# MayDomine/Burst-Attention

Hardware: NVIDIA H100
Metric: attention fwd+bwd TFLOPS/s (bs=1, H=32, d=128, bf16; seq in config, default 262144 on N > 1 GPUs, 65536 on one), aggregate over GPUs (higher is better)
Workload: dtype bf16

## Files before the change

burst-attention_b200/csrc/fwd_sm90.cu:

```cuda
#include <math.h>
#include <stdlib.h>

#include "host_common.h"
#include "sm90_ptx.cuh"

namespace ba {

constexpr int kBlockM = 128;
constexpr int kBlockN = 128;
constexpr int kKStages = 2;
constexpr int kVStages = 2;
constexpr int kBoxBytes = 128 * 64 * 2;
constexpr int kFwdThreads = 384;

struct FwdParams {
  float* o_acc;
  int64_t oacc_sb, oacc_ss, oacc_sh;
  float* lse;
  int64_t lse_sb, lse_sh;
  void* o_out;
  int64_t oout_sb, oout_ss, oout_sh;
  int B, Sq, Sk, H;
  int G;
  float scale_log2;
  const float* bias;
  int64_t bias_sb, bias_sh;
  int causal;
  int causal_off;
  int load_state;
  int store_lowp;
};

struct __align__(8) FwdBarriers {
  uint64_t q_full;
  uint64_t k_full[kKStages], k_empty[kKStages];
  uint64_t b_full[kKStages];
  uint64_t v_full[kVStages], v_empty[kVStages];
};

template <int kD>
struct FwdLayout {
  static_assert(kD == 64 || kD == 128, "head dim 64 or 128");
  static constexpr uint32_t kTileB = 128 * kD * 2;
  static constexpr int kBoxes = kD / 64;
  static constexpr uint32_t kOffQ = 0;
  static constexpr uint32_t kOffK = kTileB;
  static constexpr uint32_t kOffV = kOffK + kKStages * kTileB;
  static constexpr uint32_t kOffBias = kOffV + kVStages * kTileB;
  static constexpr uint32_t kOffBars = kOffBias + kKStages * kBlockN * 4;
  static constexpr int kSmemBytes = kOffBars + 256 ;
  static_assert(kSmemBytes <= 232448, "forward kernel exceeds 227 KiB of shared memory");
};

__device__ __forceinline__ int fwd_trip_count(int r0, const FwdParams& p) {
  if (r0 >= p.Sq) return 0;
  int r_last = min(r0 + 63, p.Sq - 1);
  int max_limit = p.causal ? min(r_last + p.causal_off, p.Sk - 1) : p.Sk - 1;
  return max_limit < 0 ? 0 : max_limit / kBlockN + 1;
}

template <bool kBF16, int kD, bool kBias>
__global__ void __launch_bounds__(kFwdThreads, 1)
fwd_chunk_kernel(const __grid_constant__ CUtensorMap tmQ, const __grid_constant__ CUtensorMap tmK,
                 const __grid_constant__ CUtensorMap tmV, const FwdParams p) {
  extern __shared__ __align__(1024) uint8_t smem_raw[];
  uint8_t* smem = smem_raw;
  if ((smem_u32(smem) & 1023u) != 0) __trap();
  using L = FwdLayout<kD>;
  constexpr uint32_t kTileBytes = L::kTileB;
  constexpr int kBoxes = L::kBoxes, kOReg = kD / 2;
  uint8_t* sQ = smem + L::kOffQ;
  uint8_t* sK = smem + L::kOffK;
  uint8_t* sV = smem + L::kOffV;
  float* sBias = reinterpret_cast<float*>(smem + L::kOffBias);
  FwdBarriers* bars = reinterpret_cast<FwdBarriers*>(smem + L::kOffBars);

  const int warp = __shfl_sync(0xffffffffu, threadIdx.x >> 5, 0);
  const int lane = threadIdx.x & 31;
  const int h = blockIdx.y, b = blockIdx.z;
  const int row0 = (p.causal ? (int)(gridDim.x - 1 - blockIdx.x) : (int)blockIdx.x) * kBlockM;
  const int n_tiles = max(fwd_trip_count(row0, p), fwd_trip_count(row0 + 64, p));

  if (threadIdx.x == 0) {
    tma_prefetch_desc(&tmQ);
    tma_prefetch_desc(&tmK);
    tma_prefetch_desc(&tmV);
    mbar_init(&bars->q_full, 1);
    for (int i = 0; i < kKStages; ++i) {
      mbar_init(&bars->k_full[i], 1);
      mbar_init(&bars->k_empty[i], 8);
      mbar_init(&bars->b_full[i], 1);
    }
    for (int i = 0; i < kVStages; ++i) {
      mbar_init(&bars->v_full[i], 1);
      mbar_init(&bars->v_empty[i], 8);
    }
    fence_mbar_init();
  }
  __syncthreads();

  if (warp < 4) {
    reg_alloc_dec<40>();
    if (warp != 0) return;
    const int hk = h / p.G;
    if (lane == 0) {
      mbar_arrive_expect_tx(&bars->q_full, kTileBytes);
      for (int half = 0; half < kBoxes; ++half)
        tma_load_4d(sQ + half * kBoxBytes, &tmQ, &bars->q_full, half * 64, h, row0, b);
    }
    for (int i = 0; i < n_tiles; ++i) {
      const int ks = i % kKStages, kph = (i / kKStages) & 1;
      mbar_wait(&bars->k_empty[ks], kph ^ 1);
      if (lane == 0) {
        mbar_arrive_expect_tx(&bars->k_full[ks], kTileBytes);
        for (int half = 0; half < kBoxes; ++half)
          tma_load_4d(sK + ks * kTileBytes + half * kBoxBytes, &tmK, &bars->k_full[ks], half * 64, hk,
                      i * kBlockN, b);
      }
      if constexpr (kBias) {
#pragma unroll
        for (int j = 0; j < 4; ++j) {
          const int key = i * kBlockN + lane + 32 * j;
          float x = 0.f;
          if (key < p.Sk) x = __ldg(p.bias + (int64_t)b * p.bias_sb + (int64_t)h * p.bias_sh + key) * kLog2e;
          sBias[ks * kBlockN + lane + 32 * j] = x;
        }
        __syncwarp();
        if (lane == 0) mbar_arrive(&bars->b_full[ks]);
      }
      if (lane == 0) {
        const int vs = i % kVStages, vph = (i / kVStages) & 1;
        mbar_wait(&bars->v_empty[vs], vph ^ 1);
        mbar_arrive_expect_tx(&bars->v_full[vs], kTileBytes);
        for (int half = 0; half < kBoxes; ++half)
          tma_load_4d(sV + vs * kTileBytes + half * kBoxBytes, &tmV, &bars->v_full[vs], half * 64, hk,
                      i * kBlockN, b);
      }
      __syncwarp();
    }
    return;
  }

  reg_alloc_inc<232>();
  const int wg = (threadIdx.x >> 7) - 1;
  const int w = warp & 3, g = lane >> 2, t = lane & 3;
  const int r_lo = row0 + wg * 64 + 16 * w + g;
  const int rows[2] = {r_lo, r_lo + 8};
  const int n_mine = fwd_trip_count(row0 + wg * 64, p);
  const float scale_log2 = p.scale_log2;
  int limit[2];
#pragma unroll
  for (int r = 0; r < 2; ++r) limit[r] = p.causal ? min(rows[r] + p.causal_off, p.Sk - 1) : p.Sk - 1;
  const int limit_min = min(limit[0], limit[1]);

  float o[kOReg];
  float m[2] = {-INFINITY, -INFINITY}, l[2] = {0.f, 0.f};
#pragma unroll
  for (int i = 0; i < kOReg; ++i) o[i] = 0.f;
  if (p.load_state) {
#pragma unroll
    for (int r = 0; r < 2; ++r) {
      if (rows[r] >= p.Sq) continue;
      const float lse_prev = p.lse[(int64_t)b * p.lse_sb + (int64_t)h * p.lse_sh + rows[r]];
      if (lse_prev != -INFINITY) {
        m[r] = lse_prev * kLog2e;
        l[r] = t == 0 ? 1.f : 0.f;
      }
      const float* src = p.o_acc + (int64_t)b * p.oacc_sb + (int64_t)rows[r] * p.oacc_ss + (int64_t)h * p.oacc_sh;
#pragma unroll
      for (int c = 0; c < kD / 8; ++c) {
        const float2 f = __ldg(reinterpret_cast<const float2*>(src + 8 * c + 2 * t));
        o[4 * c + 2 * r] = f.x;
        o[4 * c + 2 * r + 1] = f.y;
      }
    }
  }

  const uint32_t q_base = smem_u32(sQ) + wg * 64 * 128;
  mbar_wait(&bars->q_full, 0);
  for (int i = 0; i < n_tiles; ++i) {
    const int ks = i % kKStages, kph = (i / kKStages) & 1;
    const int vs = i % kVStages, vph = (i / kVStages) & 1;
    const bool work = i < n_mine;
    mbar_wait(&bars->k_full[ks], kph);
    float sc[64];
    if (work) {
      const uint32_t k_base = smem_u32(sK + ks * kTileBytes);
      wgmma_fence();
#pragma unroll
      for (int kk = 0; kk < kD / 16; ++kk) {
        const uint32_t off = (kk >> 2) * kBoxBytes + (kk & 3) * 32;
        wgmma_ss_n128<kBF16, 0, 0>(sc, make_desc(q_base + off, 16, 1024), make_desc(k_base + off, 16, 1024),
                                   kk > 0 ? 1u : 0u);
      }
      wgmma_commit();
      wgmma_wait<0>();
      fence_regs<64>(sc);
      const int key0 = i * kBlockN;
      if constexpr (kBias) {
        mbar_wait(&bars->b_full[ks], kph);
        const float* bias = sBias + ks * kBlockN;
#pragma unroll
        for (int c = 0; c < 16; ++c) {
          const float2 bb = *reinterpret_cast<const float2*>(bias + 8 * c + 2 * t);
#pragma unroll
          for (int r = 0; r < 2; ++r) {
            sc[4 * c + 2 * r] = fmaf(sc[4 * c + 2 * r], scale_log2, bb.x);
            sc[4 * c + 2 * r + 1] = fmaf(sc[4 * c + 2 * r + 1], scale_log2, bb.y);
          }
        }
      } else {
#pragma unroll
        for (int j = 0; j < 64; ++j) sc[j] *= scale_log2;
      }
      if (key0 + kBlockN - 1 > limit_min) {
#pragma unroll
        for (int c = 0; c < 16; ++c)
#pragma unroll
          for (int e = 0; e < 4; ++e)
            if (key0 + 8 * c + 2 * t + (e & 1) > limit[e >> 1]) sc[4 * c + e] = -INFINITY;
      }
    }
    __syncwarp();
    if (lane == 0) mbar_arrive(&bars->k_empty[ks]);
    if (work) {
      uint32_t pa[32];
#pragma unroll
      for (int r = 0; r < 2; ++r) {
        float mx = -INFINITY;
#pragma unroll
        for (int c = 0; c < 16; ++c) mx = fmaxf(mx, fmaxf(sc[4 * c + 2 * r], sc[4 * c + 2 * r + 1]));
        mx = fmaxf(mx, __shfl_xor_sync(0xffffffffu, mx, 1));
        mx = fmaxf(mx, __shfl_xor_sync(0xffffffffu, mx, 2));
        const float m_new = fmaxf(m[r], mx);
        const float f = (m[r] == -INFINITY) ? 0.f : ex2(m[r] - m_new);
        const float neg_m = (m_new == -INFINITY) ? 0.f : -m_new;
        m[r] = m_new;
        float sum = 0.f;
#pragma unroll
        for (int c = 0; c < 16; ++c) {
          const float p0 = ex2(sc[4 * c + 2 * r] + neg_m), p1 = ex2(sc[4 * c + 2 * r + 1] + neg_m);
          sc[4 * c + 2 * r] = p0;
          sc[4 * c + 2 * r + 1] = p1;
          sum += p0 + p1;
        }
        l[r] = l[r] * f + sum;
#pragma unroll
        for (int c = 0; c < kD / 8; ++c) {
          o[4 * c + 2 * r] *= f;
          o[4 * c + 2 * r + 1] *= f;
        }
      }
#pragma unroll
      for (int j = 0; j < 32; ++j) pa[j] = pack2<kBF16>(sc[2 * j], sc[2 * j + 1]);
      mbar_wait(&bars->v_full[vs], vph);
      const uint32_t v_base = smem_u32(sV + vs * kTileBytes);
      fence_regs<32>(pa);
      fence_regs<kOReg>(o);
      wgmma_fence();
#pragma unroll
      for (int kk = 0; kk < kBlockN / 16; ++kk) {
        const uint64_t dv = make_desc(v_base + kk * 16 * 128, kBoxBytes, 1024);
        if constexpr (kD == 128) wgmma_rs_n128<kBF16, 1>(o, pa + 4 * kk, dv, 1u);
        else wgmma_rs_n64<kBF16, 1>(o, pa + 4 * kk, dv, 1u);
      }
      wgmma_commit();
      wgmma_wait<0>();
      fence_regs<kOReg>(o);
    } else {
      mbar_wait(&bars->v_full[vs], vph);
    }
    __syncwarp();
    if (lane == 0) mbar_arrive(&bars->v_empty[vs]);
  }

#pragma unroll
  for (int r = 0; r < 2; ++r) {
    float lr = l[r];
    lr += __shfl_xor_sync(0xffffffffu, lr, 1);
    lr += __shfl_xor_sync(0xffffffffu, lr, 2);
    const int row = rows[r];
    if (row >= p.Sq) continue;
    const float inv_l = lr > 0.f ? 1.f / lr : 0.f;
    if (t == 0) p.lse[(int64_t)b * p.lse_sb + (int64_t)h * p.lse_sh + row] = lr > 0.f ? (m[r] + lg2(lr)) * kLn2 : -INFINITY;
    if (p.store_lowp) {
      uint16_t* dst = reinterpret_cast<uint16_t*>(p.o_out) + (int64_t)b * p.oout_sb + (int64_t)row * p.oout_ss +
                      (int64_t)h * p.oout_sh + 2 * t;
#pragma unroll
      for (int c = 0; c < kD / 8; ++c)
        *reinterpret_cast<uint32_t*>(dst + 8 * c) = pack2<kBF16>(o[4 * c + 2 * r] * inv_l, o[4 * c + 2 * r + 1] * inv_l);
    } else {
      float* dst = p.o_acc + (int64_t)b * p.oacc_sb + (int64_t)row * p.oacc_ss + (int64_t)h * p.oacc_sh + 2 * t;
#pragma unroll
      for (int c = 0; c < kD / 8; ++c)
        *reinterpret_cast<float2*>(dst + 8 * c) = make_float2(o[4 * c + 2 * r] * inv_l, o[4 * c + 2 * r + 1] * inv_l);
    }
  }
}


static int launch_fwd(int dtype, int D, bool bias, const CUtensorMap& tmQ, const CUtensorMap& tmK,
                      const CUtensorMap& tmV, const FwdParams& p, cudaStream_t stream) {
  const bool bf16 = dtype == BA_DTYPE_BF16;
  void (*kern)(CUtensorMap, CUtensorMap, CUtensorMap, FwdParams);
  if (bias)
    kern = D == 64 ? (bf16 ? fwd_chunk_kernel<true, 64, true> : fwd_chunk_kernel<false, 64, true>)
                   : (bf16 ? fwd_chunk_kernel<true, 128, true> : fwd_chunk_kernel<false, 128, true>);
  else
    kern = D == 64 ? (bf16 ? fwd_chunk_kernel<true, 64, false> : fwd_chunk_kernel<false, 64, false>)
                   : (bf16 ? fwd_chunk_kernel<true, 128, false> : fwd_chunk_kernel<false, 128, false>);
  const int smem = D == 64 ? FwdLayout<64>::kSmemBytes : FwdLayout<128>::kSmemBytes;
  BA_CHECK_CUDA(cudaFuncSetAttribute(kern, cudaFuncAttributeMaxDynamicSharedMemorySize, smem));
  dim3 grid((p.Sq + kBlockM - 1) / kBlockM, p.H, p.B);
  kern<<<grid, kFwdThreads, smem, stream>>>(tmQ, tmK, tmV, p);
  BA_CHECK_CUDA(cudaGetLastError());
  return BA_OK;
}

}

extern "C" int ba_fwd_chunk(ba_tensor4 q, ba_tensor4 k, ba_tensor4 v, ba_tensor4 o_acc, ba_rowstat lse,
                            ba_tensor4 o_out, int B, int Sq, int Sk, int H, int D, float scale, int mask_mode,
                            int causal_offset, int flags, int dtype, void* stream) {
  ba_rowstat none = {nullptr, 0, 0};
  return ba_fwd_chunk_bias(q, k, v, none, o_acc, lse, o_out, B, Sq, Sk, H, D, scale, mask_mode, causal_offset, flags,
                           dtype, stream);
}

extern "C" int ba_fwd_chunk_bias(ba_tensor4 q, ba_tensor4 k, ba_tensor4 v, ba_rowstat key_bias, ba_tensor4 o_acc,
                                 ba_rowstat lse, ba_tensor4 o_out, int B, int Sq, int Sk, int H, int D, float scale,
                                 int mask_mode, int causal_offset, int flags, int dtype, void* stream) {
  return ba_fwd_chunk_gqa(q, k, v, key_bias, o_acc, lse, o_out, B, Sq, Sk, H, H, D, scale, mask_mode, causal_offset,
                          flags, dtype, stream);
}

extern "C" int ba_fwd_chunk_gqa(ba_tensor4 q, ba_tensor4 k, ba_tensor4 v, ba_rowstat key_bias, ba_tensor4 o_acc,
                                ba_rowstat lse, ba_tensor4 o_out, int B, int Sq, int Sk, int H, int H_kv, int D,
                                float scale, int mask_mode, int causal_offset, int flags, int dtype, void* stream) {
  using namespace ba;
  int rc;
  if ((rc = check_chunk_args("ba_fwd_chunk", B, Sq, Sk, H, H_kv, D, scale, mask_mode, dtype))) return rc;
  BA_REQUIRE(q.ptr && k.ptr && v.ptr && lse.ptr, "ba_fwd_chunk: null q/k/v/lse");
  const bool first = flags & BA_FWD_FIRST, last = flags & BA_FWD_LAST;
  BA_REQUIRE(!last || o_out.ptr, "ba_fwd_chunk: BA_FWD_LAST needs o_out");
  BA_REQUIRE((first && last) || o_acc.ptr, "ba_fwd_chunk: fp32 state o_acc required unless FIRST|LAST");
  if (o_acc.ptr)
    BA_REQUIRE(aligned16(o_acc, 4), "ba_fwd_chunk: o_acc must be 16-byte aligned with strides multiple of 4 elements");
  if (o_out.ptr)
    BA_REQUIRE(aligned16(o_out, 2), "ba_fwd_chunk: o_out must be 16-byte aligned with strides multiple of 8 elements");

  CUtensorMap tmQ, tmK, tmV;
  const CUtensorMapDataType dt = lowp_dtype(dtype);
  if ((rc = make_tensor_map(&tmQ, q, B, Sq, H, D, dt, 2, 64, kBlockM, true))) return rc;
  if ((rc = make_tensor_map(&tmK, k, B, Sk, H_kv, D, dt, 2, 64, kBlockN, true))) return rc;
  if ((rc = make_tensor_map(&tmV, v, B, Sk, H_kv, D, dt, 2, 64, kBlockN, true))) return rc;

  FwdParams p;
  p.o_acc = static_cast<float*>(o_acc.ptr);
  p.oacc_sb = o_acc.stride_b, p.oacc_ss = o_acc.stride_s, p.oacc_sh = o_acc.stride_h;
  p.lse = lse.ptr;
  p.lse_sb = lse.stride_b, p.lse_sh = lse.stride_h;
  p.o_out = o_out.ptr;
  p.oout_sb = o_out.stride_b, p.oout_ss = o_out.stride_s, p.oout_sh = o_out.stride_h;
  p.B = B, p.Sq = Sq, p.Sk = Sk, p.H = H;
  p.G = H / H_kv;
  p.scale_log2 = scale * kLog2e;
  p.causal = mask_mode == BA_MASK_CAUSAL;
  p.causal_off = causal_offset;
  p.load_state = first ? 0 : 1;
  p.store_lowp = last ? 1 : 0;
  p.bias = key_bias.ptr, p.bias_sb = key_bias.stride_b, p.bias_sh = key_bias.stride_h;
  return launch_fwd(dtype, D, key_bias.ptr != nullptr, tmQ, tmK, tmV, p, static_cast<cudaStream_t>(stream));
}
```

burst-attention_b200/csrc/sm90_ptx.cuh:

```cuda
#pragma once
#include <cuda.h>
#include <cuda_bf16.h>
#include <cuda_fp16.h>
#include <cuda_runtime.h>
#include <stdint.h>

namespace ba {

#define BA_DEVICE __device__ __forceinline__

BA_DEVICE uint32_t smem_u32(const void* p) {
  return static_cast<uint32_t>(__cvta_generic_to_shared(p));
}
constexpr float kLog2e = 1.4426950408889634f;
constexpr float kLn2 = 0.6931471805599453f;
BA_DEVICE float ex2(float x) {
  float y;
  asm("ex2.approx.ftz.f32 %0, %1;" : "=f"(y) : "f"(x));
  return y;
}
BA_DEVICE float lg2(float x) {
  float y;
  asm("lg2.approx.ftz.f32 %0, %1;" : "=f"(y) : "f"(x));
  return y;
}
template <int N>
BA_DEVICE void reg_alloc_inc() {
  asm volatile("setmaxnreg.inc.sync.aligned.u32 %0;" ::"n"(N));
}
template <int N>
BA_DEVICE void reg_alloc_dec() {
  asm volatile("setmaxnreg.dec.sync.aligned.u32 %0;" ::"n"(N));
}

BA_DEVICE void mbar_init(uint64_t* bar, uint32_t count) {
  asm volatile("mbarrier.init.shared::cta.b64 [%0], %1;" ::"r"(smem_u32(bar)), "r"(count));
}
BA_DEVICE void fence_mbar_init() { asm volatile("fence.mbarrier_init.release.cluster;" ::: "memory"); }
BA_DEVICE void mbar_arrive(uint64_t* bar) {
  asm volatile("mbarrier.arrive.shared::cta.b64 _, [%0];" ::"r"(smem_u32(bar)) : "memory");
}
BA_DEVICE void mbar_arrive_expect_tx(uint64_t* bar, uint32_t bytes) {
  asm volatile("mbarrier.arrive.expect_tx.shared::cta.b64 _, [%0], %1;" ::"r"(smem_u32(bar)), "r"(bytes)
               : "memory");
}
BA_DEVICE bool mbar_try_wait(uint64_t* bar, uint32_t parity) {
  uint32_t ok;
  asm volatile(
      "{\n\t.reg .pred p;\n\t"
      "mbarrier.try_wait.parity.shared::cta.b64 p, [%1], %2;\n\t"
      "selp.u32 %0, 1, 0, p;\n\t}\n"
      : "=r"(ok)
      : "r"(smem_u32(bar)), "r"(parity)
      : "memory");
  return ok != 0;
}
BA_DEVICE uint64_t global_ns() {
  uint64_t t;
  asm volatile("mov.u64 %0, %%globaltimer;" : "=l"(t));
  return t;
}
BA_DEVICE void mbar_wait(uint64_t* bar, uint32_t parity) {
  if (mbar_try_wait(bar, parity)) return;
#ifdef BA_NO_WATCHDOG
  while (!mbar_try_wait(bar, parity)) {
  }
#else
  const uint64_t t0 = global_ns();
#pragma unroll 1
  for (;;) {
#pragma unroll 1
    for (int i = 0; i < 1024; ++i)
      if (mbar_try_wait(bar, parity)) return;
    if (global_ns() - t0 > 30000000000ull) break;
  }
  __trap();
#endif
}

BA_DEVICE void fence_proxy_async_smem() { asm volatile("fence.proxy.async.shared::cta;" ::: "memory"); }
BA_DEVICE void named_bar_sync(uint32_t id, uint32_t nthreads) {
  asm volatile("bar.sync %0, %1;" ::"r"(id), "r"(nthreads) : "memory");
}

BA_DEVICE void tma_prefetch_desc(const CUtensorMap* m) {
  asm volatile("prefetch.tensormap [%0];" ::"l"(reinterpret_cast<uint64_t>(m)) : "memory");
}
BA_DEVICE void tma_load_4d(void* smem_dst, const CUtensorMap* m, uint64_t* bar, int c0, int c1, int c2,
                           int c3) {
  asm volatile(
      "cp.async.bulk.tensor.4d.shared::cluster.global.mbarrier::complete_tx::bytes"
      " [%0], [%1, {%3, %4, %5, %6}], [%2];"
      :
      : "r"(smem_u32(smem_dst)), "l"(reinterpret_cast<uint64_t>(m)), "r"(smem_u32(bar)), "r"(c0), "r"(c1),
        "r"(c2), "r"(c3)
      : "memory");
}
BA_DEVICE void tma_reduce_add_4d(const CUtensorMap* m, const void* smem_src, int c0, int c1, int c2, int c3) {
  asm volatile(
      "cp.reduce.async.bulk.tensor.4d.global.shared::cta.add.tile.bulk_group [%0, {%2, %3, %4, %5}], [%1];"
      :
      : "l"(reinterpret_cast<uint64_t>(m)), "r"(smem_u32(smem_src)), "r"(c0), "r"(c1), "r"(c2), "r"(c3)
      : "memory");
}
BA_DEVICE void tma_store_commit() { asm volatile("cp.async.bulk.commit_group;" ::: "memory"); }
template <int N>
BA_DEVICE void tma_store_wait_read() {
  asm volatile("cp.async.bulk.wait_group.read %0;" ::"n"(N) : "memory");
}
template <int N>
BA_DEVICE void tma_store_wait() {
  asm volatile("cp.async.bulk.wait_group %0;" ::"n"(N) : "memory");
}

BA_DEVICE uint64_t make_desc(uint32_t smem_addr, uint32_t lbo_bytes, uint32_t sbo_bytes) {
  uint64_t d = 0;
  d |= static_cast<uint64_t>((smem_addr & 0x3FFFF) >> 4);
  d |= static_cast<uint64_t>((lbo_bytes >> 4) & 0x3FFF) << 16;
  d |= static_cast<uint64_t>((sbo_bytes >> 4) & 0x3FFF) << 32;
  d |= static_cast<uint64_t>(1) << 62;
  return d;
}

BA_DEVICE void wgmma_fence() { asm volatile("wgmma.fence.sync.aligned;" ::: "memory"); }
BA_DEVICE void wgmma_commit() { asm volatile("wgmma.commit_group.sync.aligned;" ::: "memory"); }
template <int N>
BA_DEVICE void wgmma_wait() {
  asm volatile("wgmma.wait_group.sync.aligned %0;" ::"n"(N) : "memory");
}
template <int N>
BA_DEVICE void fence_regs(float* r) {
#pragma unroll
  for (int i = 0; i < N; ++i) asm volatile("" : "+f"(r[i])::"memory");
}
template <int N>
BA_DEVICE void fence_regs(uint32_t* r) {
#pragma unroll
  for (int i = 0; i < N; ++i) asm volatile("" : "+r"(r[i])::"memory");
}

#define BA_WGMMA_ACC_64(d) "+f"(d[0]), "+f"(d[1]), "+f"(d[2]), "+f"(d[3]), "+f"(d[4]), "+f"(d[5]), "+f"(d[6]), "+f"(d[7]), "+f"(d[8]), "+f"(d[9]), "+f"(d[10]), "+f"(d[11]), "+f"(d[12]), "+f"(d[13]), "+f"(d[14]), "+f"(d[15]), "+f"(d[16]), "+f"(d[17]), "+f"(d[18]), "+f"(d[19]), "+f"(d[20]), "+f"(d[21]), "+f"(d[22]), "+f"(d[23]), "+f"(d[24]), "+f"(d[25]), "+f"(d[26]), "+f"(d[27]), "+f"(d[28]), "+f"(d[29]), "+f"(d[30]), "+f"(d[31])
#define BA_WGMMA_ACC_128(d) BA_WGMMA_ACC_64(d), "+f"(d[32]), "+f"(d[33]), "+f"(d[34]), "+f"(d[35]), "+f"(d[36]), "+f"(d[37]), "+f"(d[38]), "+f"(d[39]), "+f"(d[40]), "+f"(d[41]), "+f"(d[42]), "+f"(d[43]), "+f"(d[44]), "+f"(d[45]), "+f"(d[46]), "+f"(d[47]), "+f"(d[48]), "+f"(d[49]), "+f"(d[50]), "+f"(d[51]), "+f"(d[52]), "+f"(d[53]), "+f"(d[54]), "+f"(d[55]), "+f"(d[56]), "+f"(d[57]), "+f"(d[58]), "+f"(d[59]), "+f"(d[60]), "+f"(d[61]), "+f"(d[62]), "+f"(d[63])
#define BA_WGMMA_REGS_64 "%0,%1,%2,%3,%4,%5,%6,%7,%8,%9,%10,%11,%12,%13,%14,%15,%16,%17,%18,%19,%20,%21,%22,%23,%24,%25,%26,%27,%28,%29,%30,%31"
#define BA_WGMMA_REGS_128 BA_WGMMA_REGS_64 ",%32,%33,%34,%35,%36,%37,%38,%39,%40,%41,%42,%43,%44,%45,%46,%47,%48,%49,%50,%51,%52,%53,%54,%55,%56,%57,%58,%59,%60,%61,%62,%63"
#define BA_WGMMA_SS(N, TY, A, B, SC, TA, TB)                                                     \
  asm volatile("{\n\t.reg .pred p;\n\t"                                                        \
               "setp.ne.b32 p, %" #SC ", 0;\n\t"                                               \
               "wgmma.mma_async.sync.aligned.m64n" #N "k16.f32." TY "." TY " "                 \
               "{" BA_WGMMA_REGS_##N "}, "                                                      \
               "%" #A ", %" #B ", p, 1, 1, %" #TA ", %" #TB ";\n\t}\n"                         \
               : BA_WGMMA_ACC_##N(d)                                                            \
               : "l"(a_desc), "l"(b_desc), "r"(scale_d), "n"(kTA), "n"(kTB))
#define BA_WGMMA_RS(N, TY, A0, A1, A2, A3, B, SC, TB)                                            \
  asm volatile("{\n\t.reg .pred p;\n\t"                                                        \
               "setp.ne.b32 p, %" #SC ", 0;\n\t"                                               \
               "wgmma.mma_async.sync.aligned.m64n" #N "k16.f32." TY "." TY " "                 \
               "{" BA_WGMMA_REGS_##N "}, "                                                      \
               "{%" #A0 ",%" #A1 ",%" #A2 ",%" #A3 "}, %" #B ", p, 1, 1, %" #TB ";\n\t}\n"     \
               : BA_WGMMA_ACC_##N(d)                                                            \
               : "r"(a[0]), "r"(a[1]), "r"(a[2]), "r"(a[3]), "l"(b_desc), "r"(scale_d), "n"(kTB))

template <bool kBF16, int kTA, int kTB>
BA_DEVICE void wgmma_ss_n64(float* d, uint64_t a_desc, uint64_t b_desc, uint32_t scale_d) {
  if constexpr (kBF16) BA_WGMMA_SS(64, "bf16", 32, 33, 34, 35, 36);
  else BA_WGMMA_SS(64, "f16", 32, 33, 34, 35, 36);
}
template <bool kBF16, int kTB>
BA_DEVICE void wgmma_rs_n64(float* d, const uint32_t* a, uint64_t b_desc, uint32_t scale_d) {
  if constexpr (kBF16) BA_WGMMA_RS(64, "bf16", 32, 33, 34, 35, 36, 37, 38);
  else BA_WGMMA_RS(64, "f16", 32, 33, 34, 35, 36, 37, 38);
}
template <bool kBF16, int kTA, int kTB>
BA_DEVICE void wgmma_ss_n128(float* d, uint64_t a_desc, uint64_t b_desc, uint32_t scale_d) {
  if constexpr (kBF16) BA_WGMMA_SS(128, "bf16", 64, 65, 66, 67, 68);
  else BA_WGMMA_SS(128, "f16", 64, 65, 66, 67, 68);
}
template <bool kBF16, int kTB>
BA_DEVICE void wgmma_rs_n128(float* d, const uint32_t* a, uint64_t b_desc, uint32_t scale_d) {
  if constexpr (kBF16) BA_WGMMA_RS(128, "bf16", 64, 65, 66, 67, 68, 69, 70);
  else BA_WGMMA_RS(128, "f16", 64, 65, 66, 67, 68, 69, 70);
}

template <bool kBF16>
BA_DEVICE uint32_t pack2(float lo, float hi) {
  if constexpr (kBF16) {
    __nv_bfloat162 v = __floats2bfloat162_rn(lo, hi);
    return *reinterpret_cast<uint32_t*>(&v);
  } else {
    __half2 v = __floats2half2_rn(lo, hi);
    return *reinterpret_cast<uint32_t*>(&v);
  }
}

}
```

Measured before the change: 470.8.

## Pipeline forward QK and PV wgmma with warpgroup ping-pong scheduling

Restructures the forward consumer loop so that the S=QK^T wgmma for tile i is issued together with the PV wgmma for tile i-1, and softmax runs while the PV GEMM is in flight. It adds named-barrier ping-pong between the two consumer warpgroups so their tensor-core issue phases alternate. Q is loaded once into registers and the QK GEMM uses the register-A variant. The aim is to hide softmax latency behind tensor-core work, at the cost of more register pressure and more complex synchronisation, including peeled first and last iterations.

```diff
diff --git a/burst-attention_b200/csrc/fwd_sm90.cu b/burst-attention_b200/csrc/fwd_sm90.cu
--- a/burst-attention_b200/csrc/fwd_sm90.cu
+++ b/burst-attention_b200/csrc/fwd_sm90.cu
@@ -147,6 +147,7 @@
   const int r_lo = row0 + wg * 64 + 16 * w + g;
   const int rows[2] = {r_lo, r_lo + 8};
   const int n_mine = fwd_trip_count(row0 + wg * 64, p);
+  const int n_pp = min(n_mine, fwd_trip_count(row0 + (1 - wg) * 64, p));
   const float scale_log2 = p.scale_log2;
   int limit[2];
 #pragma unroll
@@ -176,102 +177,162 @@
     }
   }
 
-  const uint32_t q_base = smem_u32(sQ) + wg * 64 * 128;
-  mbar_wait(&bars->q_full, 0);
-  for (int i = 0; i < n_tiles; ++i) {
+  float sc[64];
+  uint32_t qa[kD / 4];
+  uint32_t pa[32];
+  float f[2];
+
+  auto issue_s = [&](int i) {
+    const uint32_t k_base = smem_u32(sK + (i % kKStages) * kTileBytes);
+#pragma unroll
+    for (int kk = 0; kk < kD / 16; ++kk) {
+      const uint32_t off = (kk >> 2) * kBoxBytes + (kk & 3) * 32;
+      wgmma_rs_n128<kBF16, 0>(sc, qa + 4 * kk, make_desc(k_base + off, 16, 1024), kk > 0 ? 1u : 0u);
+    }
+    wgmma_commit();
+  };
+  auto issue_pv = [&](int i) {
+    const uint32_t v_base = smem_u32(sV + (i % kVStages) * kTileBytes);
+#pragma unroll
+    for (int kk = 0; kk < kBlockN / 16; ++kk) {
+      const uint64_t dv = make_desc(v_base + kk * 16 * 128, kBoxBytes, 1024);
+      if constexpr (kD == 128) wgmma_rs_n128<kBF16, 1>(o, pa + 4 * kk, dv, 1u);
+      else wgmma_rs_n64<kBF16, 1>(o, pa + 4 * kk, dv, 1u);
+    }
+    wgmma_commit();
+  };
+  auto scores = [&](int i) {
     const int ks = i % kKStages, kph = (i / kKStages) & 1;
-    const int vs = i % kVStages, vph = (i / kVStages) & 1;
-    const bool work = i < n_mine;
-    mbar_wait(&bars->k_full[ks], kph);
-    float sc[64];
-    if (work) {
-      const uint32_t k_base = smem_u32(sK + ks * kTileBytes);
-      wgmma_fence();
-#pragma unroll
-      for (int kk = 0; kk < kD / 16; ++kk) {
-        const uint32_t off = (kk >> 2) * kBoxBytes + (kk & 3) * 32;
-        wgmma_ss_n128<kBF16, 0, 0>(sc, make_desc(q_base + off, 16, 1024), make_desc(k_base + off, 16, 1024),
-                                   kk > 0 ? 1u : 0u);
-      }
-      wgmma_commit();
-      wgmma_wait<0>();
-      fence_regs<64>(sc);
-      const int key0 = i * kBlockN;
-      if constexpr (kBias) {
-        mbar_wait(&bars->b_full[ks], kph);
-        const float* bias = sBias + ks * kBlockN;
-#pragma unroll
-        for (int c = 0; c < 16; ++c) {
-          const float2 bb = *reinterpret_cast<const float2*>(bias + 8 * c + 2 * t);
-#pragma unroll
-          for (int r = 0; r < 2; ++r) {
-            sc[4 * c + 2 * r] = fmaf(sc[4 * c + 2 * r], scale_log2, bb.x);
-            sc[4 * c + 2 * r + 1] = fmaf(sc[4 * c + 2 * r + 1], scale_log2, bb.y);
-          }
+    const int key0 = i * kBlockN;
+    if constexpr (kBias) {
+      mbar_wait(&bars->b_full[ks], kph);
+      const float* bias = sBias + ks * kBlockN;
+#pragma unroll
+      for (int c = 0; c < 16; ++c) {
+        const float2 bb = *reinterpret_cast<const float2*>(bias + 8 * c + 2 * t);
+#pragma unroll
+        for (int r = 0; r < 2; ++r) {
+          sc[4 * c + 2 * r] = fmaf(sc[4 * c + 2 * r], scale_log2, bb.x);
+          sc[4 * c + 2 * r + 1] = fmaf(sc[4 * c + 2 * r + 1], scale_log2, bb.y);
         }
-      } else {
-#pragma unroll
-        for (int j = 0; j < 64; ++j) sc[j] *= scale_log2;
-      }
-      if (key0 + kBlockN - 1 > limit_min) {
-#pragma unroll
-        for (int c = 0; c < 16; ++c)
-#pragma unroll
-          for (int e = 0; e < 4; ++e)
-            if (key0 + 8 * c + 2 * t + (e & 1) > limit[e >> 1]) sc[4 * c + e] = -INFINITY;
-      }
+      }
+    } else {
+#pragma unroll
+      for (int j = 0; j < 64; ++j) sc[j] *= scale_log2;
+    }
+    if (key0 + kBlockN - 1 > limit_min) {
+#pragma unroll
+      for (int c = 0; c < 16; ++c)
+#pragma unroll
+        for (int e = 0; e < 4; ++e)
+          if (key0 + 8 * c + 2 * t + (e & 1) > limit[e >> 1]) sc[4 * c + e] = -INFINITY;
     }
     __syncwarp();
     if (lane == 0) mbar_arrive(&bars->k_empty[ks]);
-    if (work) {
-      uint32_t pa[32];
-#pragma unroll
-      for (int r = 0; r < 2; ++r) {
-        float mx = -INFINITY;
-#pragma unroll
-        for (int c = 0; c < 16; ++c) mx = fmaxf(mx, fmaxf(sc[4 * c + 2 * r], sc[4 * c + 2 * r + 1]));
-        mx = fmaxf(mx, __shfl_xor_sync(0xffffffffu, mx, 1));
-        mx = fmaxf(mx, __shfl_xor_sync(0xffffffffu, mx, 2));
-        const float m_new = fmaxf(m[r], mx);
-        const float f = (m[r] == -INFINITY) ? 0.f : ex2(m[r] - m_new);
-        const float neg_m = (m_new == -INFINITY) ? 0.f : -m_new;
-        m[r] = m_new;
-        float sum = 0.f;
-#pragma unroll
-        for (int c = 0; c < 16; ++c) {
-          const float p0 = ex2(sc[4 * c + 2 * r] + neg_m), p1 = ex2(sc[4 * c + 2 * r + 1] + neg_m);
-          sc[4 * c + 2 * r] = p0;
-          sc[4 * c + 2 * r + 1] = p1;
-          sum += p0 + p1;
-        }
-        l[r] = l[r] * f + sum;
-#pragma unroll
-        for (int c = 0; c < kD / 8; ++c) {
-          o[4 * c + 2 * r] *= f;
-          o[4 * c + 2 * r + 1] *= f;
-        }
-      }
-#pragma unroll
-      for (int j = 0; j < 32; ++j) pa[j] = pack2<kBF16>(sc[2 * j], sc[2 * j + 1]);
-      mbar_wait(&bars->v_full[vs], vph);
-      const uint32_t v_base = smem_u32(sV + vs * kTileBytes);
+  };
+  auto softmax = [&]() {
+#pragma unroll
+    for (int r = 0; r < 2; ++r) {
+      float mx = -INFINITY;
+#pragma unroll
+      for (int c = 0; c < 16; ++c) mx = fmaxf(mx, fmaxf(sc[4 * c + 2 * r], sc[4 * c + 2 * r + 1]));
+      mx = fmaxf(mx, __shfl_xor_sync(0xffffffffu, mx, 1));
+      mx = fmaxf(mx, __shfl_xor_sync(0xffffffffu, mx, 2));
+      const float m_new = fmaxf(m[r], mx);
+      f[r] = (m[r] == -INFINITY) ? 0.f : ex2(m[r] - m_new);
+      const float neg_m = (m_new == -INFINITY) ? 0.f : -m_new;
+      m[r] = m_new;
+      float sum = 0.f;
+#pragma unroll
+      for (int c = 0; c < 16; ++c) {
+        const float p0 = ex2(sc[4 * c + 2 * r] + neg_m), p1 = ex2(sc[4 * c + 2 * r + 1] + neg_m);
+        sc[4 * c + 2 * r] = p0;
+        sc[4 * c + 2 * r + 1] = p1;
+        sum += p0 + p1;
+      }
+      l[r] = l[r] * f[r] + sum;
+    }
+  };
+  auto rescale_pack = [&]() {
+#pragma unroll
+    for (int r = 0; r < 2; ++r)
+#pragma unroll
+      for (int c = 0; c < kD / 8; ++c) {
+        o[4 * c + 2 * r] *= f[r];
+        o[4 * c + 2 * r + 1] *= f[r];
+      }
+#pragma unroll
+    for (int j = 0; j < 32; ++j) pa[j] = pack2<kBF16>(sc[2 * j], sc[2 * j + 1]);
+  };
+  auto release_v = [&](int i) {
+    __syncwarp();
+    if (lane == 0) mbar_arrive(&bars->v_empty[i % kVStages]);
+  };
+  auto turn_begin = [&](int i) {
+    if (i < n_pp) named_bar_sync(1 + wg, 256);
+  };
+  auto turn_end = [&](int i) {
+    if (i < n_pp && (wg == 0 || i + 1 < n_pp)) named_bar_arrive(2 - wg, 256);
+  };
+
+  if (wg == 1 && n_pp > 0) named_bar_arrive(1, 256);
+  mbar_wait(&bars->q_full, 0);
+#pragma unroll
+  for (int kk = 0; kk < kD / 16; ++kk)
+#pragma unroll
+    for (int j = 0; j < 4; ++j) {
+      const int row = wg * 64 + 16 * w + g + 8 * (j & 1), chunk = 2 * (kk & 3) + (j >> 1);
+      qa[4 * kk + j] = *reinterpret_cast<const uint32_t*>(sQ + (kk >> 2) * kBoxBytes + row * 128 +
+                                                          ((chunk ^ g) << 4) + 4 * t);
+    }
+  if (n_mine > 0) {
+    mbar_wait(&bars->k_full[0], 0);
+    turn_begin(0);
+    wgmma_fence();
+    issue_s(0);
+    turn_end(0);
+    wgmma_wait<0>();
+    fence_regs<64>(sc);
+    scores(0);
+    softmax();
+    rescale_pack();
+    for (int i = 1; i < n_mine; ++i) {
+      mbar_wait(&bars->k_full[i % kKStages], (i / kKStages) & 1);
+      mbar_wait(&bars->v_full[(i - 1) % kVStages], ((i - 1) / kVStages) & 1);
+      turn_begin(i);
       fence_regs<32>(pa);
       fence_regs<kOReg>(o);
       wgmma_fence();
-#pragma unroll
-      for (int kk = 0; kk < kBlockN / 16; ++kk) {
-        const uint64_t dv = make_desc(v_base + kk * 16 * 128, kBoxBytes, 1024);
-        if constexpr (kD == 128) wgmma_rs_n128<kBF16, 1>(o, pa + 4 * kk, dv, 1u);
-        else wgmma_rs_n64<kBF16, 1>(o, pa + 4 * kk, dv, 1u);
-      }
-      wgmma_commit();
+      issue_s(i);
+      issue_pv(i - 1);
+      turn_end(i);
+      wgmma_wait<1>();
+      fence_regs<64>(sc);
+      scores(i);
+      softmax();
       wgmma_wait<0>();
       fence_regs<kOReg>(o);
-    } else {
-      mbar_wait(&bars->v_full[vs], vph);
-    }
+      fence_regs<32>(pa);
+      release_v(i - 1);
+      rescale_pack();
+    }
+    const int last = n_mine - 1;
+    mbar_wait(&bars->v_full[last % kVStages], (last / kVStages) & 1);
+    fence_regs<32>(pa);
+    fence_regs<kOReg>(o);
+    wgmma_fence();
+    issue_pv(last);
+    wgmma_wait<0>();
+    fence_regs<kOReg>(o);
+    fence_regs<32>(pa);
+    release_v(last);
+  }
+  for (int i = n_mine; i < n_tiles; ++i) {
+    mbar_wait(&bars->k_full[i % kKStages], (i / kKStages) & 1);
     __syncwarp();
-    if (lane == 0) mbar_arrive(&bars->v_empty[vs]);
+    if (lane == 0) mbar_arrive(&bars->k_empty[i % kKStages]);
+    mbar_wait(&bars->v_full[i % kVStages], (i / kVStages) & 1);
+    release_v(i);
   }
 
 #pragma unroll
diff --git a/burst-attention_b200/csrc/sm90_ptx.cuh b/burst-attention_b200/csrc/sm90_ptx.cuh
--- a/burst-attention_b200/csrc/sm90_ptx.cuh
+++ b/burst-attention_b200/csrc/sm90_ptx.cuh
@@ -81,6 +81,9 @@
 BA_DEVICE void fence_proxy_async_smem() { asm volatile("fence.proxy.async.shared::cta;" ::: "memory"); }
 BA_DEVICE void named_bar_sync(uint32_t id, uint32_t nthreads) {
   asm volatile("bar.sync %0, %1;" ::"r"(id), "r"(nthreads) : "memory");
+}
+BA_DEVICE void named_bar_arrive(uint32_t id, uint32_t nthreads) {
+  asm volatile("bar.arrive %0, %1;" ::"r"(id), "r"(nthreads) : "memory");
 }
 
 BA_DEVICE void tma_prefetch_desc(const CUtensorMap* m) {
```

Result: faster. 479.0, median of 6 (+1.7%).

## Software-pipeline forward loop: overlap next QK^T with current PV wgmma

Applied to the files above, without the earlier changes.

Restructures the consumer loop of the SM90 forward kernel so the S=QK^T wgmma for tile i is issued together with the PV wgmma for tile i-1. The softmax for tile i then runs while the PV GEMM is still in flight, in the style of FlashAttention-3 intra-warpgroup overlap. It also skips the O rescale when no row max changed (warp-uniform check) and uses a per-warpgroup mask threshold. The cost is more live registers (sc, pa and o at once) and more complex barrier release ordering.

```diff
diff --git a/burst-attention_b200/csrc/fwd_sm90.cu b/burst-attention_b200/csrc/fwd_sm90.cu
--- a/burst-attention_b200/csrc/fwd_sm90.cu
+++ b/burst-attention_b200/csrc/fwd_sm90.cu
@@ -142,7 +142,7 @@
   }
 
   reg_alloc_inc<232>();
-  const int wg = (threadIdx.x >> 7) - 1;
+  const int wg = (warp >> 2) - 1;
   const int w = warp & 3, g = lane >> 2, t = lane & 3;
   const int r_lo = row0 + wg * 64 + 16 * w + g;
   const int rows[2] = {r_lo, r_lo + 8};
@@ -151,7 +151,6 @@
   int limit[2];
 #pragma unroll
   for (int r = 0; r < 2; ++r) limit[r] = p.causal ? min(rows[r] + p.causal_off, p.Sk - 1) : p.Sk - 1;
-  const int limit_min = min(limit[0], limit[1]);
 
   float o[kOReg];
   float m[2] = {-INFINITY, -INFINITY}, l[2] = {0.f, 0.f};
@@ -177,101 +176,149 @@
   }
 
   const uint32_t q_base = smem_u32(sQ) + wg * 64 * 128;
+  const int limit_wg = p.causal ? min(row0 + wg * 64 + p.causal_off, p.Sk - 1) : p.Sk - 1;
+
+  auto issue_s = [&](float* sc, int ks) {
+    const uint32_t k_base = smem_u32(sK + ks * kTileBytes);
+#pragma unroll
+    for (int kk = 0; kk < kD / 16; ++kk) {
+      const uint32_t off = (kk >> 2) * kBoxBytes + (kk & 3) * 32;
+      wgmma_ss_n128<kBF16, 0, 0>(sc, make_desc(q_base + off, 16, 1024), make_desc(k_base + off, 16, 1024),
+                                 kk > 0 ? 1u : 0u);
+    }
+    wgmma_commit();
+  };
+  auto issue_pv = [&](const uint32_t* pa, int vs) {
+    const uint32_t v_base = smem_u32(sV + vs * kTileBytes);
+#pragma unroll
+    for (int kk = 0; kk < kBlockN / 16; ++kk) {
+      const uint64_t dv = make_desc(v_base + kk * 16 * 128, kBoxBytes, 1024);
+      if constexpr (kD == 128) wgmma_rs_n128<kBF16, 1>(o, pa + 4 * kk, dv, 1u);
+      else wgmma_rs_n64<kBF16, 1>(o, pa + 4 * kk, dv, 1u);
+    }
+    wgmma_commit();
+  };
+  auto scale_mask = [&](float* sc, int i, int ks) {
+    if constexpr (kBias) {
+      const float* bias = sBias + ks * kBlockN;
+#pragma unroll
+      for (int c = 0; c < 16; ++c) {
+        const float2 bb = *reinterpret_cast<const float2*>(bias + 8 * c + 2 * t);
+#pragma unroll
+        for (int r = 0; r < 2; ++r) {
+          sc[4 * c + 2 * r] = fmaf(sc[4 * c + 2 * r], scale_log2, bb.x);
+          sc[4 * c + 2 * r + 1] = fmaf(sc[4 * c + 2 * r + 1], scale_log2, bb.y);
+        }
+      }
+    } else {
+#pragma unroll
+      for (int j = 0; j < 64; ++j) sc[j] *= scale_log2;
+    }
+    const int key0 = i * kBlockN;
+    if (key0 + kBlockN - 1 > limit_wg) {
+#pragma unroll
+      for (int c = 0; c < 16; ++c)
+#pragma unroll
+        for (int e = 0; e < 4; ++e)
+          sc[4 * c + e] = key0 + 8 * c + 2 * t + (e & 1) > limit[e >> 1] ? -INFINITY : sc[4 * c + e];
+    }
+  };
+  auto softmax = [&](float* sc, float* f) {
+#pragma unroll
+    for (int r = 0; r < 2; ++r) {
+      float mx = -INFINITY;
+#pragma unroll
+      for (int c = 0; c < 16; ++c) mx = fmaxf(mx, fmaxf(sc[4 * c + 2 * r], sc[4 * c + 2 * r + 1]));
+      mx = fmaxf(mx, __shfl_xor_sync(0xffffffffu, mx, 1));
+      mx = fmaxf(mx, __shfl_xor_sync(0xffffffffu, mx, 2));
+      const float m_new = fmaxf(m[r], mx);
+      f[r] = (m[r] == -INFINITY) ? 0.f : ex2(m[r] - m_new);
+      const float neg_m = (m_new == -INFINITY) ? 0.f : -m_new;
+      m[r] = m_new;
+      float sum = 0.f;
+#pragma unroll
+      for (int c = 0; c < 16; ++c) {
+        const float p0 = ex2(sc[4 * c + 2 * r] + neg_m), p1 = ex2(sc[4 * c + 2 * r + 1] + neg_m);
+        sc[4 * c + 2 * r] = p0;
+        sc[4 * c + 2 * r + 1] = p1;
+        sum += p0 + p1;
+      }
+      l[r] = l[r] * f[r] + sum;
+    }
+  };
+  auto rescale_pack = [&](const float* f, const float* sc, uint32_t* pa) {
+    if (__any_sync(0xffffffffu, f[0] != 1.f || f[1] != 1.f)) {
+#pragma unroll
+      for (int r = 0; r < 2; ++r)
+#pragma unroll
+        for (int c = 0; c < kD / 8; ++c) {
+          o[4 * c + 2 * r] *= f[r];
+          o[4 * c + 2 * r + 1] *= f[r];
+        }
+    }
+#pragma unroll
+    for (int j = 0; j < 32; ++j) pa[j] = pack2<kBF16>(sc[2 * j], sc[2 * j + 1]);
+  };
+  auto release = [&](uint64_t* bar) {
+    __syncwarp();
+    if (lane == 0) mbar_arrive(bar);
+  };
+
   mbar_wait(&bars->q_full, 0);
-  for (int i = 0; i < n_tiles; ++i) {
-    const int ks = i % kKStages, kph = (i / kKStages) & 1;
-    const int vs = i % kVStages, vph = (i / kVStages) & 1;
-    const bool work = i < n_mine;
-    mbar_wait(&bars->k_full[ks], kph);
-    float sc[64];
-    if (work) {
-      const uint32_t k_base = smem_u32(sK + ks * kTileBytes);
-      wgmma_fence();
-#pragma unroll
-      for (int kk = 0; kk < kD / 16; ++kk) {
-        const uint32_t off = (kk >> 2) * kBoxBytes + (kk & 3) * 32;
-        wgmma_ss_n128<kBF16, 0, 0>(sc, make_desc(q_base + off, 16, 1024), make_desc(k_base + off, 16, 1024),
-                                   kk > 0 ? 1u : 0u);
-      }
-      wgmma_commit();
-      wgmma_wait<0>();
-      fence_regs<64>(sc);
-      const int key0 = i * kBlockN;
-      if constexpr (kBias) {
-        mbar_wait(&bars->b_full[ks], kph);
-        const float* bias = sBias + ks * kBlockN;
-#pragma unroll
-        for (int c = 0; c < 16; ++c) {
-          const float2 bb = *reinterpret_cast<const float2*>(bias + 8 * c + 2 * t);
-#pragma unroll
-          for (int r = 0; r < 2; ++r) {
-            sc[4 * c + 2 * r] = fmaf(sc[4 * c + 2 * r], scale_log2, bb.x);
-            sc[4 * c + 2 * r + 1] = fmaf(sc[4 * c + 2 * r + 1], scale_log2, bb.y);
-          }
-        }
-      } else {
-#pragma unroll
-        for (int j = 0; j < 64; ++j) sc[j] *= scale_log2;
-      }
-      if (key0 + kBlockN - 1 > limit_min) {
-#pragma unroll
-        for (int c = 0; c < 16; ++c)
-#pragma unroll
-          for (int e = 0; e < 4; ++e)
-            if (key0 + 8 * c + 2 * t + (e & 1) > limit[e >> 1]) sc[4 * c + e] = -INFINITY;
-      }
-    }
-    __syncwarp();
-    if (lane == 0) mbar_arrive(&bars->k_empty[ks]);
-    if (work) {
-      uint32_t pa[32];
-#pragma unroll
-      for (int r = 0; r < 2; ++r) {
-        float mx = -INFINITY;
-#pragma unroll
-        for (int c = 0; c < 16; ++c) mx = fmaxf(mx, fmaxf(sc[4 * c + 2 * r], sc[4 * c + 2 * r + 1]));
-        mx = fmaxf(mx, __shfl_xor_sync(0xffffffffu, mx, 1));
-        mx = fmaxf(mx, __shfl_xor_sync(0xffffffffu, mx, 2));
-        const float m_new = fmaxf(m[r], mx);
-        const float f = (m[r] == -INFINITY) ? 0.f : ex2(m[r] - m_new);
-        const float neg_m = (m_new == -INFINITY) ? 0.f : -m_new;
-        m[r] = m_new;
-        float sum = 0.f;
-#pragma unroll
-        for (int c = 0; c < 16; ++c) {
-          const float p0 = ex2(sc[4 * c + 2 * r] + neg_m), p1 = ex2(sc[4 * c + 2 * r + 1] + neg_m);
-          sc[4 * c + 2 * r] = p0;
-          sc[4 * c + 2 * r + 1] = p1;
-          sum += p0 + p1;
-        }
-        l[r] = l[r] * f + sum;
-#pragma unroll
-        for (int c = 0; c < kD / 8; ++c) {
-          o[4 * c + 2 * r] *= f;
-          o[4 * c + 2 * r + 1] *= f;
-        }
-      }
-#pragma unroll
-      for (int j = 0; j < 32; ++j) pa[j] = pack2<kBF16>(sc[2 * j], sc[2 * j + 1]);
+  float sc[64], f[2];
+  uint32_t pa[32];
+  if (n_mine > 0) {
+    mbar_wait(&bars->k_full[0], 0);
+    if constexpr (kBias) mbar_wait(&bars->b_full[0], 0);
+    wgmma_fence();
+    issue_s(sc, 0);
+    wgmma_wait<0>();
+    fence_regs<64>(sc);
+    scale_mask(sc, 0, 0);
+    release(&bars->k_empty[0]);
+    softmax(sc, f);
+    for (int i = 1; i < n_mine; ++i) {
+      const int ks = i % kKStages, kph = (i / kKStages) & 1;
+      const int vs = (i - 1) % kVStages, vph = ((i - 1) / kVStages) & 1;
+      if (i > 1) release(&bars->v_empty[(i - 2) % kVStages]);
+      rescale_pack(f, sc, pa);
+      mbar_wait(&bars->k_full[ks], kph);
+      if constexpr (kBias) mbar_wait(&bars->b_full[ks], kph);
       mbar_wait(&bars->v_full[vs], vph);
-      const uint32_t v_base = smem_u32(sV + vs * kTileBytes);
       fence_regs<32>(pa);
       fence_regs<kOReg>(o);
       wgmma_fence();
-#pragma unroll
-      for (int kk = 0; kk < kBlockN / 16; ++kk) {
-        const uint64_t dv = make_desc(v_base + kk * 16 * 128, kBoxBytes, 1024);
-        if constexpr (kD == 128) wgmma_rs_n128<kBF16, 1>(o, pa + 4 * kk, dv, 1u);
-        else wgmma_rs_n64<kBF16, 1>(o, pa + 4 * kk, dv, 1u);
-      }
-      wgmma_commit();
+      issue_s(sc, ks);
+      issue_pv(pa, vs);
+      wgmma_wait<1>();
+      fence_regs<64>(sc);
+      scale_mask(sc, i, ks);
+      release(&bars->k_empty[ks]);
+      softmax(sc, f);
+      fence_regs<64>(sc);
       wgmma_wait<0>();
       fence_regs<kOReg>(o);
-    } else {
-      mbar_wait(&bars->v_full[vs], vph);
-    }
-    __syncwarp();
-    if (lane == 0) mbar_arrive(&bars->v_empty[vs]);
+      fence_regs<32>(pa);
+    }
+    const int vs = (n_mine - 1) % kVStages, vph = ((n_mine - 1) / kVStages) & 1;
+    if (n_mine > 1) release(&bars->v_empty[(n_mine - 2) % kVStages]);
+    rescale_pack(f, sc, pa);
+    mbar_wait(&bars->v_full[vs], vph);
+    fence_regs<32>(pa);
+    fence_regs<kOReg>(o);
+    wgmma_fence();
+    issue_pv(pa, vs);
+    wgmma_wait<0>();
+    fence_regs<kOReg>(o);
+    release(&bars->v_empty[vs]);
+  }
+  for (int i = n_mine; i < n_tiles; ++i) {
+    const int ks = i % kKStages, kph = (i / kKStages) & 1;
+    const int vs = i % kVStages, vph = (i / kVStages) & 1;
+    mbar_wait(&bars->k_full[ks], kph);
+    release(&bars->k_empty[ks]);
+    mbar_wait(&bars->v_full[vs], vph);
+    release(&bars->v_empty[vs]);
   }
 
 #pragma unroll
```

Result: no change. 467.9 before, 469.1 after, median of 6 (+0.3%).
